# CrawlScript/tf_geometric

Measured on AMD Instinct MI355X. Metric: aggregated edges/sec + achieved HBM GB/s, GCN layer, higher is better.
Workload: dtype f32

## Files before the change

### tf_geometric_amd/csrc/tfgx_reduce.hip

```cpp
#include "tfgx_common.h"
#include <cfloat>
#include <cstdio>
#include <cstdlib>

namespace tfgx {
namespace {

template <int G>
__device__ __forceinline__ int bcast_i(int v, int j)
{
    if constexpr (G == 64) return __builtin_amdgcn_readlane(v, j);
    else return __shfl(v, j, G);
}
template <int G>
__device__ __forceinline__ float bcast_f(float v, int j)
{
    if constexpr (G == 64) return __int_as_float(__builtin_amdgcn_readlane(__float_as_int(v), j));
    else return __shfl(v, j, G);
}

struct KArgs {
    const int32_t* row_begin;
    const int32_t* row_end;
    int64_t rp_stride;
// ... 286 lines not shown
                            if constexpr (IS_MAX) {
                                const float m = WEIGHTED ? xv[u][k][v] * ww[u] : xv[u][k][v];
                                if constexpr (TRACK) {
                                    if (live) track_step(k, v, m, base + j + u);
                                }
                                const float t = fmaxf(acc[k][v], m);
                                acc[k][v] = live ? t : acc[k][v];
                            } else {
                                const float t = WEIGHTED ? fmaf(ww[u], xv[u][k][v], acc[k][v]) : acc[k][v] + xv[u][k][v];
                                acc[k][v] = live ? t : acc[k][v];
                            }
                        }
                }
            }
            }
        }

        const float sc = a.self_coef ? a.self_coef[r] : 0.0f;
        bool mismatch = false;
        float divisor = 1.0f;
        if (a.op == TFGX_MEAN) {
            const int cnt = a.mean_count ? a.mean_count[r] : (e - s);
            divisor = float(cnt > 1 ? cnt : 1);
        }
#pragma unroll
        for (int k = 0; k < CH; ++k) {
            if (!cvalid[k]) continue;
            float res[VEC];
#pragma unroll
            for (int v = 0; v < VEC; ++v) res[v] = acc[k][v];
            float* op = a.out + r * a.ldo + coff[k];
            float mine[TRACK ? VEC : 1], before[TRACK ? VEC : 1];
            if (a.accumulate) {
                float prev[VEC];
                load_vec<VEC>(op, prev);
#pragma unroll
                for (int v = 0; v < VEC; ++v) {
                    if constexpr (TRACK) { mine[v] = res[v]; before[v] = prev[v]; }
                    res[v] = IS_MAX ? fmaxf(prev[v], res[v]) : prev[v] + res[v];
                }
            }
            if (a.self_coef) {
                float xself[VEC];
                if constexpr (VERIFY) {
                    float xlay[VEC];
                    load_vec<VEC>(a.verify_x + r * a.ld_verify_x + coff[k], xself);
                    load_vec<VEC>(xs[k] + r * xsl[k], xlay);
#pragma unroll
                    for (int v = 0; v < VEC; ++v) mismatch = mismatch || __float_as_uint(xself[v]) != __float_as_uint(xlay[v]);
                } else if constexpr (SPLIT) load_vec<VEC>(xs[k] + r * xsl[k], xself);
                else load_vec<VEC>(a.x + r * a.ldx + coff[k], xself);
#pragma unroll
                for (int v = 0; v < VEC; ++v) {
                    if constexpr (IS_MAX) res[v] = fmaxf(res[v], sc * xself[v]);
                    else res[v] = fmaf(sc, xself[v], res[v]);
                }
            }
            if (a.op == TFGX_MEAN) {
#pragma unroll
                for (int v = 0; v < VEC; ++v) res[v] = res[v] / divisor;
            }
            if (a.add_x) {
                float xa[VEC];
                load_vec<VEC>(a.add_x + r * a.ld_add + coff[k], xa);
#pragma unroll
                for (int v = 0; v < VEC; ++v) res[v] = xa[v] + res[v];
            }
            if (a.bias) {
                float b[VEC];
                load_vec<VEC>(a.bias + coff[k], b);
#pragma unroll
                for (int v = 0; v < VEC; ++v) res[v] += b[v];
            }
#pragma unroll
            for (int v = 0; v < VEC; ++v) res[v] = apply_act(res[v], a.act);
            store_vec<VEC>(op, res);
            if constexpr (TRACK) {
                const int s_rel = a.track_row_begin ? a.track_row_begin[r * a.rp_stride] : s;
                uint32_t pk[VEC];
#pragma unroll
                for (int v = 0; v < VEC; ++v) {
                    const uint32_t c = uint32_t(tcnt[k][v] < 65535 ? tcnt[k][v] : 65535);
                    pk[v] = (c << 16) | (tpos[k][v] < 0 ? 0xFFFFu : uint32_t(tpos[k][v] - s_rel) & 0xFFFFu);
                }
                uint32_t* tp = a.track + r * a.ld_track + coff[k];
                if (a.accumulate) {
                    uint32_t old[VEC];
                    if constexpr (VEC == 4) {
                        const uint4 o4 = *reinterpret_cast<const uint4*>(tp);
                        old[0] = o4.x; old[1] = o4.y; old[2] = o4.z; old[3] = o4.w;
                    } else {
#pragma unroll
                        for (int v = 0; v < VEC; ++v) old[v] = tp[v];
                    }
#pragma unroll
                    for (int v = 0; v < VEC; ++v) {
                        const uint32_t oc = old[v] >> 16, nc = pk[v] >> 16;
                        const uint32_t sum = oc + nc < 65535u ? oc + nc : 65535u;
                        const bool none_before = (old[v] & 0xFFFFu) == 0xFFFFu && oc == 0u;
                        if (mine[v] > before[v] || none_before) {  }
                        else if (mine[v] == before[v] && nc > 0u) pk[v] = (sum << 16) | (old[v] & 0xFFFFu);
                        else pk[v] = old[v];
                    }
                }
                if constexpr (VEC == 4) *reinterpret_cast<uint4*>(tp) = make_uint4(pk[0], pk[1], pk[2], pk[3]);
                else {
#pragma unroll
                    for (int v = 0; v < VEC; ++v) tp[v] = pk[v];
                }
            }
        }
        if constexpr (VERIFY) {
            if (mismatch) *a.verify_word = 1u;
        }
    }
}

inline size_t dummy_lds_bytes()
{
    static long v = -1;
    if (v < 0) {
        const char* e = getenv("TFGX_REDUCE_DUMMY_LDS");
        v = (e != nullptr && atol(e) > 0) ? atol(e) : 0;
    }
    return size_t(v);
}

inline int reduce_grid_cap()
{
    static int cap = 0;
    if (cap == 0) {
        const char* e = getenv("TFGX_REDUCE_GRID_CAP");
        cap = (e != nullptr && atoi(e) > 0) ? atoi(e) : TFGX_REDUCE_GRID_CAP_DEFAULT;
    }
    return cap;
}

inline bool wide_blocks_enabled()
{
    static int v = -1;
    if (v < 0) {
        const char* e = getenv("TFGX_REDUCE_WIDE_BLOCKS");
        v = (e != nullptr && atoi(e) == 0) ? 0 : 1;
    }
    return v != 0;
}
inline int wide_g256()
{
    static int v = -1;
    if (v < 0) {
        const char* e = getenv("TFGX_REDUCE_WIDE_G256");
        v = (e != nullptr && atoi(e) == 16) ? 16 : 32;
    }
    return v;
}

template <int VEC, int G, int CH, int U = 0>
int launch_cfg(const KArgs& a, bool is_max, bool weighted, int ny, hipStream_t stream)
{
    constexpr int ROWS_PER_BLOCK = kBlock / G;
    dim3 grid(grid_for(a.n_dst, ROWS_PER_BLOCK, CH >= 2 ? (reduce_grid_cap() < 4096 ? reduce_grid_cap() : 4096) : reduce_grid_cap()), ny, 1);
    dim3 block(kBlock, 1, 1);
    if constexpr (VEC == 4 && CH == 1) {
        if (a.x_tail != nullptr && a.verify_x != nullptr) {
            if (is_max) {
                if (weighted) seg_reduce_verify_kernel<VEC, G, CH, true, true, U><<<grid, block, dummy_lds_bytes(), stream>>>(a);
                else seg_reduce_verify_kernel<VEC, G, CH, true, false, U><<<grid, block, dummy_lds_bytes(), stream>>>(a);
            } else {
                if (weighted) seg_reduce_verify_kernel<VEC, G, CH, false, true, U><<<grid, block, dummy_lds_bytes(), stream>>>(a);
                else seg_reduce_verify_kernel<VEC, G, CH, false, false, U><<<grid, block, dummy_lds_bytes(), stream>>>(a);
            }
            TFGX_LAUNCH_CHECK("seg_reduce_verify_kernel");
            return TFGX_OK;
        }
        if (a.x_tail != nullptr) {
            if (is_max) {
                if (weighted) seg_reduce_kernel<VEC, G, CH, true, true, true, false, U><<<grid, block, dummy_lds_bytes(), stream>>>(a);
                else seg_reduce_kernel<VEC, G, CH, true, false, true, false, U><<<grid, block, dummy_lds_bytes(), stream>>>(a);
            } else {
                if (weighted) seg_reduce_kernel<VEC, G, CH, false, true, true, false, U><<<grid, block, dummy_lds_bytes(), stream>>>(a);
                else seg_reduce_kernel<VEC, G, CH, false, false, true, false, U><<<grid, block, dummy_lds_bytes(), stream>>>(a);
            }
            TFGX_LAUNCH_CHECK("seg_reduce_kernel<split>");
            return TFGX_OK;
        }
    }
    if (a.x_tail != nullptr) {
        set_error("tfgx_segment_reduce_f32: x_tail needs 16-byte aligned rows and F <= 256");
        return TFGX_ERR_INVALID_ARG;
    }
    if (a.track != nullptr) {
        if constexpr (VEC == 4 && CH == 1) {
            if (weighted) seg_reduce_kernel<VEC, G, CH, true, true, false, true, U><<<grid, block, dummy_lds_bytes(), stream>>>(a);
            else seg_reduce_kernel<VEC, G, CH, true, false, false, true, U><<<grid, block, dummy_lds_bytes(), stream>>>(a);
            TFGX_LAUNCH_CHECK("seg_reduce_kernel<track>");
            return TFGX_OK;
        }
        set_error("tfgx_segment_reduce_f32: track needs 16-byte aligned rows, F % 4 == 0, of F <= 256 columns or of whole 128-byte lines");
        return TFGX_ERR_INVALID_ARG;
    }
    if (is_max) {
        if (weighted) seg_reduce_kernel<VEC, G, CH, true, true, false, false, U><<<grid, block, dummy_lds_bytes(), stream>>>(a);
        else seg_reduce_kernel<VEC, G, CH, true, false, false, false, U><<<grid, block, dummy_lds_bytes(), stream>>>(a);
    } else {
        if (weighted) seg_reduce_kernel<VEC, G, CH, false, true, false, false, U><<<grid, block, dummy_lds_bytes(), stream>>>(a);
        else seg_reduce_kernel<VEC, G, CH, false, false, false, false, U><<<grid, block, dummy_lds_bytes(), stream>>>(a);
    }
    TFGX_LAUNCH_CHECK("seg_reduce_kernel");
    return TFGX_OK;
}

template <typename K>
int resident_grid(K k, int* blocks)
{
    if (*blocks == 0) {
        int dev = 0, cus = 0, per_cu = 0;
        if (hipGetDevice(&dev) != hipSuccess ||
            hipDeviceGetAttribute(&cus, hipDeviceAttributeMultiprocessorCount, dev) != hipSuccess || cus <= 0)
            cus = 256;
        if (hipOccupancyMaxActiveBlocksPerMultiprocessor(&per_cu, k, kBlock, 0) != hipSuccess || per_cu <= 0) per_cu = 1;
        *blocks = cus * per_cu;
    }
    return *blocks;
}

template <int G>
int launch_repair_g(const KArgs& a, bool is_max, bool weighted, hipStream_t stream)
{
    static int blocks[4] = {0, 0, 0, 0};
    auto go = [&](auto kernel, int slot) {
        kernel<<<dim3(resident_grid(kernel, &blocks[slot]), 1, 1), dim3(kBlock, 1, 1), 0, stream>>>(a);
    };
    if (is_max) {
        if (weighted) go(seg_reduce_repair_kernel<4, G, 1, true, true>, 0);
        else go(seg_reduce_repair_kernel<4, G, 1, true, false>, 1);
    } else {
        if (weighted) go(seg_reduce_repair_kernel<4, G, 1, false, true>, 2);
        else go(seg_reduce_repair_kernel<4, G, 1, false, false>, 3);
    }
    TFGX_LAUNCH_CHECK("seg_reduce_repair_kernel");
    return TFGX_OK;
}

int launch_repair(const KArgs& a, int G, bool is_max, bool weighted, hipStream_t stream)
{
    switch (G) {
        case 4: return launch_repair_g<4>(a, is_max, weighted, stream);
        case 8: return launch_repair_g<8>(a, is_max, weighted, stream);
        case 16: return launch_repair_g<16>(a, is_max, weighted, stream);
        case 32: return launch_repair_g<32>(a, is_max, weighted, stream);
        default: return launch_repair_g<64>(a, is_max, weighted, stream);
    }
}

struct GroupShape { int G, CH, NY, U; };

inline GroupShape group_shape(const KArgs& a, int vec)
{
    const int lanes = (a.F + vec - 1) / vec;
    if (vec == 4 && a.F >= 128 && a.F % 32 == 0 && a.ldx % 32 == 0 && aligned_to(a.x, 128) && a.x_tail == nullptr &&
        a.wide_blocks >= 0 && (a.wide_blocks > 0 || wide_blocks_enabled())) {
        const int g = a.F == 256 ? wide_g256() : 16;
        return GroupShape{g, 1, (lanes + g - 1) / g, 16};
    }
    if (lanes <= 4) return GroupShape{4, 1, 1, 0};
    if (lanes <= 8) return GroupShape{8, 1, 1, 0};
    if (lanes <= 16) return GroupShape{16, 1, 1, 0};
    if (lanes <= 32) return GroupShape{32, 1, 1, 0};
    if (lanes <= 64) return GroupShape{64, 1, 1, 0};
    if (lanes <= 128) return GroupShape{64, 2, 1, 0};
    const int per = 64 * 4;
    return GroupShape{64, 4, (lanes + per - 1) / per, 0};
}

template <int VEC>
int launch_vec(const KArgs& a, bool is_max, bool weighted, hipStream_t stream)
{
    const GroupShape g = group_shape(a, VEC);
    if constexpr (VEC == 4) {
        if (g.U == 16 && g.G == 16) return launch_cfg<4, 16, 1, 16>(a, is_max, weighted, g.NY, stream);
        if (g.U == 16 && g.G == 32) return launch_cfg<4, 32, 1, 16>(a, is_max, weighted, g.NY, stream);
    }
    if (g.CH == 1) {
        switch (g.G) {
            case 4: return launch_cfg<VEC, 4, 1>(a, is_max, weighted, 1, stream);
            case 8: return launch_cfg<VEC, 8, 1>(a, is_max, weighted, 1, stream);
            case 16: return launch_cfg<VEC, 16, 1>(a, is_max, weighted, 1, stream);
            case 32: return launch_cfg<VEC, 32, 1>(a, is_max, weighted, 1, stream);
            default: return launch_cfg<VEC, 64, 1>(a, is_max, weighted, 1, stream);
        }
    }
    if (g.CH == 2) return launch_cfg<VEC, 64, 2>(a, is_max, weighted, 1, stream);
    return launch_cfg<VEC, 64, 4>(a, is_max, weighted, g.NY, stream);
}

struct HubArgs {
    const int32_t* hub_rows;
    const int32_t* hub_chunk_ptr;
    const float* scratch;
    int64_t n_hub;
    KArgs k;
};

__global__ __launch_bounds__(kBlock) void hub_finalize_kernel(const HubArgs h)
{
    const KArgs& a = h.k;
    const bool is_max = a.op == TFGX_MAX;
    int64_t t = blockIdx.x * int64_t(kBlock) + threadIdx.x;
    const int64_t stride = int64_t(gridDim.x) * kBlock;
    const int64_t total = h.n_hub * a.F;
    for (; t < total; t += stride) {
        const int64_t i = t / a.F;
        const int j = int(t - i * a.F);
        const int64_t r = h.hub_rows[i];
        float res = is_max ? -FLT_MAX : 0.0f;
        constexpr int HB = 16;
        int c = h.hub_chunk_ptr[i];
        const int c_end = h.hub_chunk_ptr[i + 1];
        const float* sp = h.scratch + int64_t(c) * a.F + j;
        for (; c + HB <= c_end; c += HB, sp += int64_t(HB) * a.F) {
            float v[HB];
#pragma unroll
            for (int u = 0; u < HB; ++u) v[u] = __builtin_nontemporal_load(sp + int64_t(u) * a.F);
#pragma unroll
            for (int u = 0; u < HB; ++u) res = is_max ? fmaxf(res, v[u]) : res + v[u];
        }
        for (; c < c_end; ++c, sp += a.F) {
            const float v = *sp;
            res = is_max ? fmaxf(res, v) : res + v;
        }
        float* op = a.out + r * a.ldo + j;
        if (a.accumulate) res = is_max ? fmaxf(*op, res) : *op + res;
        if (a.self_coef) {
            const float xv = (a.x_tail != nullptr && j >= a.f_main) ? a.x_tail[r * a.ld_tail + (j - a.f_main)]
                                                                    : a.x[r * a.ldx + j];
            res = is_max ? fmaxf(res, a.self_coef[r] * xv) : fmaf(a.self_coef[r], xv, res);
        }
        if (a.op == TFGX_MEAN) {
            const int cnt = a.mean_count ? a.mean_count[r]
                                         : (a.row_end[r * a.rp_stride] - a.row_begin[r * a.rp_stride]);
            res = res / float(cnt > 1 ? cnt : 1);
        }
        if (a.add_x) res = a.add_x[r * a.ld_add + j] + res;
        if (a.bias) res += a.bias[j];
        *op = apply_act(res, a.act);
    }
}

int launch_any(const KArgs& a, int vec, bool is_max, bool weighted, hipStream_t stream)
{
    if (vec == 4) return launch_vec<4>(a, is_max, weighted, stream);
    if (vec == 2) return launch_vec<2>(a, is_max, weighted, stream);
    return launch_vec<1>(a, is_max, weighted, stream);
}

}
}

using namespace tfgx;

static int vector_width(const tfgx_reduce_args* p)
{
    auto ok = [&](int vec) {
        const size_t al = sizeof(float) * vec;
        bool good = (p->F % vec == 0) && (p->ldx % vec == 0) && (p->ldo % vec == 0) && aligned_to(p->x, al) &&
                    aligned_to(p->out, al);
        if (p->add_x) good = good && (p->ld_add % vec == 0) && aligned_to(p->add_x, al);
        if (p->bias) good = good && aligned_to(p->bias, al);
        return good;
    };
    int vec = ok(4) ? 4 : (ok(2) ? 2 : 1);
    while (vec > 1 && p->F / vec < 8) vec /= 2;
    return vec;
}

extern "C" int tfgx_segment_reduce_describe(const tfgx_reduce_args* p, char* buf, size_t buf_bytes)
{
    TFGX_REQUIRE(p != nullptr && buf != nullptr && buf_bytes > 0, "null argument");
    const int vec = vector_width(p);
    KArgs a;
    a.F = int32_t(p->F); a.ldx = p->ldx; a.x = p->x; a.x_tail = p->x_tail; a.wide_blocks = p->wide_blocks;
    const GroupShape g = group_shape(a, vec);
    const bool split = p->x_tail != nullptr && vec == 4 && g.CH == 1;
    if (p->verify && split) {
        const bool fused = p->self_coef != nullptr && p->n_verify == p->n_dst;
        snprintf(buf, buf_bytes, "%sseg_reduce_verify_kernel<%d, %d, %d, %s, %s, %d> + seg_reduce_repair_kernel",
                 fused ? "" : "split_rows_compare_kernel + ", vec, g.G, g.CH, p->op == TFGX_MAX ? "true" : "false",
                 p->w ? "true" : "false", g.U);
        return TFGX_OK;
    }
    snprintf(buf, buf_bytes, "seg_reduce_kernel<%d, %d, %d, %s, %s, %s, %s, %d>", vec, g.G, g.CH, p->op == TFGX_MAX ? "true" : "false",
             p->w ? "true" : "false", split ? "true" : "false", p->track ? "true" : "false", g.U);
    return TFGX_OK;
}

extern "C" int tfgx_segment_reduce_f32(const tfgx_reduce_args* p, tfgx_stream_t stream_)
{
    TFGX_RANGE();
    TFGX_REQUIRE(p != nullptr, "args is null");
    TFGX_REQUIRE(p->n_dst >= 0 && p->F >= 1 && p->F < (int64_t(1) << 30), "bad n_dst / F");
    TFGX_REQUIRE(p->op == TFGX_SUM || p->op == TFGX_MEAN || p->op == TFGX_MAX, "bad op");
    TFGX_REQUIRE(p->act == TFGX_ACT_NONE || p->act == TFGX_ACT_RELU, "bad act");
    if (p->n_dst == 0) return TFGX_OK;
    TFGX_REQUIRE(p->row_begin && p->row_end && p->out && p->x, "null pointer");
    TFGX_REQUIRE((p->ldx >= p->F || p->x_tail) && p->ldo >= p->F, "leading dimension < F");
    TFGX_REQUIRE(p->rp_stride >= 1, "rp_stride < 1");
    TFGX_REQUIRE(!(p->add_x) || p->ld_add >= p->F, "ld_add < F");

    KArgs a;
    a.row_begin = p->row_begin; a.row_end = p->row_end; a.rp_stride = p->rp_stride;
    a.col = p->col; a.w = p->w; a.n_dst = p->n_dst; a.x = p->x; a.ldx = p->ldx; a.F = int32_t(p->F);
    a.col0 = 0; a.out = p->out; a.ldo = p->ldo; a.op = p->op; a.act = p->act; a.accumulate = p->accumulate;
    a.self_coef = p->self_coef; a.bias = p->bias; a.add_x = p->add_x; a.ld_add = p->ld_add;
    a.mean_count = p->mean_count;
    a.hub_threshold = 0;
    a.x_tail = p->x_tail; a.ld_tail = p->ld_tail; a.f_main = int32_t(p->f_main);
    a.edge_tail = p->edge_tail; a.ld_edge_tail = p->ld_edge_tail;
    a.wide_blocks = p->wide_blocks;
    a.row_order = p->row_order;
    a.track = p->track; a.ld_track = p->ld_track; a.track_row_begin = p->track_row_begin;
    if (p->track) {
        TFGX_REQUIRE(p->op == TFGX_MAX && !p->self_coef && !p->x_tail && p->hub_threshold == 0 && !p->bias && !p->add_x &&
                         p->act == TFGX_ACT_NONE,
                     "track: plain TFGX_MAX launches only (no self_coef / bias / activation / split rows / hub lists)");
        TFGX_REQUIRE(p->ld_track >= p->F && p->ld_track % 4 == 0 && aligned_to(p->track, 16), "track: bad leading dimension / alignment");
    }
    TFGX_REQUIRE(p->edge_tail == nullptr ||
                     (p->x_tail != nullptr && p->ld_edge_tail >= p->F - p->f_main && p->ld_edge_tail % 4 == 0 &&
                      aligned_to(p->edge_tail, 16)),
                 "edge_tail needs the split-row layout (x_tail) and 16-byte aligned rows");
    if (p->x_tail) {
        TFGX_REQUIRE(p->f_main > 0 && p->f_main < p->F && p->f_main % 4 == 0 && (p->F - p->f_main) % 4 == 0 &&
                         p->ld_tail >= p->F - p->f_main && p->ld_tail % 4 == 0 && p->ldx >= p->f_main &&
                         aligned_to(p->x_tail, 16),
                     "bad split-row layout (f_main / ld_tail / alignment)");
    }
    const bool use_hub = p->hub_threshold > 0 && p->n_hub_rows > 0;
    if (use_hub) {
        TFGX_REQUIRE(p->hub_rows && p->hub_chunk_ptr && p->hub_chunk_begin && p->hub_chunk_end && p->hub_scratch &&
                         p->n_hub_chunks > 0,
                     "hub rows given without chunk lists / scratch");
        a.hub_threshold = p->hub_threshold;
    }

    const bool is_max = p->op == TFGX_MAX;
    const bool weighted = p->w != nullptr;
    hipStream_t stream = as_stream(stream_);

    int vec = vector_width(p);
    a.verify_x = nullptr; a.ld_verify_x = 0; a.verify_word = nullptr;
    if (p->verify) {
        TFGX_REQUIRE(p->x_tail && p->edge_tail && p->verify_x && p->verify_word && p->n_verify >= 0,
                     "verify: needs the split layout with edge_tail, verify_x and verify_word");
        TFGX_REQUIRE(!p->accumulate && !p->track && !use_hub, "verify: no accumulate / track / hub lists");
        TFGX_REQUIRE(p->ld_verify_x >= p->F && p->ld_verify_x % 4 == 0 && aligned_to(p->verify_x, 16) &&
                         aligned_to(p->verify_word, 4),
                     "verify: verify_x needs 16-byte aligned rows");
        const GroupShape g = group_shape(a, vec);
        TFGX_REQUIRE(vec == 4 && g.CH == 1, "verify: the split layout needs 16-byte aligned rows and F <= 256");
        a.verify_word = p->verify_word;
        if (p->self_coef != nullptr && p->n_verify == p->n_dst) {
            a.verify_x = p->verify_x;
            a.ld_verify_x = p->ld_verify_x;
        } else if (p->n_verify > 0) {
            split_rows_compare_kernel<<<grid_for(p->n_verify * (p->F / 4), kBlock, 8192), kBlock, 0, stream>>>(
                p->verify_x, p->ld_verify_x, p->n_verify, int(p->F), int(p->f_main), p->x, p->ldx, p->x_tail, p->ld_tail,
                p->verify_word);
            TFGX_LAUNCH_CHECK("split_rows_compare_kernel");
        }
        int rc = launch_any(a, vec, is_max, weighted, stream);
        if (rc != TFGX_OK) return rc;
        KArgs r = a;
        r.x = p->verify_x; r.ldx = p->ld_verify_x; r.x_tail = nullptr; r.ld_tail = 0; r.f_main = 0;
        r.edge_tail = nullptr; r.ld_edge_tail = 0; r.verify_x = nullptr; r.ld_verify_x = 0;
        return launch_repair(r, g.G, is_max, weighted, stream);
    }
    int rc = launch_any(a, vec, is_max, weighted, stream);
    if (rc != TFGX_OK || !use_hub) return rc;

    KArgs c = a;
    c.row_begin = p->hub_chunk_begin; c.row_end = p->hub_chunk_end; c.rp_stride = 1;
    c.n_dst = p->n_hub_chunks; c.out = p->hub_scratch; c.ldo = p->F;
    c.op = is_max ? TFGX_MAX : TFGX_SUM; c.act = TFGX_ACT_NONE; c.accumulate = 0;
    c.self_coef = nullptr; c.bias = nullptr; c.add_x = nullptr; c.mean_count = nullptr; c.hub_threshold = 0;
    c.row_order = nullptr; c.track = nullptr; c.track_row_begin = nullptr;
    const bool sok = (p->F % 4 == 0) && aligned_to(p->hub_scratch, 16) && (p->ldx % 4 == 0) && aligned_to(p->x, 16);
    const bool sok2 = (p->F % 2 == 0) && aligned_to(p->hub_scratch, 8) && (p->ldx % 2 == 0) && aligned_to(p->x, 8);
    rc = launch_any(c, sok ? 4 : (sok2 ? 2 : 1), is_max, weighted, stream);
    if (rc != TFGX_OK) return rc;
    HubArgs h;
    h.hub_rows = p->hub_rows; h.hub_chunk_ptr = p->hub_chunk_ptr; h.scratch = p->hub_scratch;
    h.n_hub = p->n_hub_rows; h.k = a;
    hub_finalize_kernel<<<grid_for(p->n_hub_rows * p->F, kBlock), kBlock, 0, stream>>>(h);
    TFGX_LAUNCH_CHECK("hub_finalize_kernel");
    return TFGX_OK;
}
```

### tf_geometric_amd/plan.py

```python
import ctypes

import torch

from . import _lib as L

CACHE_KEY_PLAN = "tfgx_csr_plan"


class CsrPlan(object):

    def __init__(self, row_ptr, col, perm, n_dst, n_src, num_edges):
        self.row_ptr = row_ptr
        self.col = col
        self.perm = perm
        self.n_dst = int(n_dst)
        self.n_src = int(n_src)
        self.num_edges = int(num_edges)
        self._edge_index = None
        self._transposed = None
        self._hub = None

    @staticmethod
    def build(edge_index, n_dst, n_src=None):
        lib = L.require_gpu()
# ... 389 lines not shown
CACHE_KEY_STATIC_ROWS = "tfgx_static_rows"


STATIC_STATS = {"hits": 0, "builds": 0}


def _static_key(x, plan):
    return (x.data_ptr(), x._version, int(x.shape[0]), int(x.shape[1]), id(plan))


def _build_static_rows(x, plan, cache):
    n, F = int(x.shape[0]), int(x.shape[1])
    rows, nbytes = None, 0
    if SplitRows.wanted(n, F):
        rows = SplitRows.from_dense(x).with_edge_tail(plan)
        nbytes = 4 * (rows.main.numel() + rows.tail.numel() + rows.edge_tail.numel())
    cache[CACHE_KEY_STATIC_ROWS] = (_static_key(x, plan), rows, x, plan, nbytes)
    STATIC_STATS["builds"] += 1
    return rows, nbytes


CACHE_KEY_STATIC_AGG = "tfgx_static_aggregated"


def prepare_static_features(x, edge_index, cache, num_nodes=None, cache_aggregation=False):
    if cache is None:
        raise ValueError("prepare_static_features needs the graph's cache dict")
    x = L.as_f32(x)
    if x.dim() != 2 or not x.is_contiguous():
        raise ValueError("static features must be a contiguous [num_nodes, num_features] float32 tensor")
    n = int(x.shape[0]) if num_nodes is None else int(num_nodes)
    plan = edge_index if isinstance(edge_index, CsrPlan) else CsrPlan.from_cache(edge_index, n, int(x.shape[0]), cache)
    cache[CACHE_KEY_STATIC] = x
    cache.pop(CACHE_KEY_STATIC_AUTO, None)
    if cache_aggregation:
        cache[CACHE_KEY_STATIC_AGG] = {}
    else:
        cache.pop(CACHE_KEY_STATIC_AGG, None)
    rows, nbytes = _build_static_rows(x, plan, cache)
    F = int(x.shape[1])
    return dict(bytes=nbytes, layout="edge_tail" if rows is not None else "dense", tensor=x,
                f_main=(F // 32) * 32 if rows is not None else F, f_tail=F % 32 if rows is not None else 0)


def release_static_features(cache):
    cache.pop(CACHE_KEY_STATIC_AUTO, None)
    cache.pop(CACHE_KEY_STATIC, None)
    cache.pop(CACHE_KEY_STATIC_ROWS, None)
    cache.pop(CACHE_KEY_STATIC_AGG, None)


def _declared_static(x, cache):
    if cache is None or not isinstance(x, torch.Tensor):
        return False
    opt = cache.get(CACHE_KEY_STATIC, None)
    if opt is None or opt is False or not isinstance(opt, torch.Tensor):
        return False
    return (opt.data_ptr() == x.data_ptr() and opt.shape == x.shape and opt.dtype == x.dtype
            and opt.stride() == x.stride())


def static_aggregate(x, plan, cache, op, w_csr=None, self_coef=None):
    store = cache.get(CACHE_KEY_STATIC_AGG) if cache is not None else None
    if store is None or not _declared_static(x, cache):
        return None
    if any(t is not None and t.requires_grad for t in (x, w_csr, self_coef)):
        return None
    if torch.cuda.is_current_stream_capturing():
        return None
    ident = lambda t: None if t is None else (t.data_ptr(), t._version, int(t.numel()))
    key = (_static_key(x, plan), ident(w_csr), ident(self_coef))
    hit = store.get(op)
    if hit is not None and hit[0] == key:
        STATIC_STATS["agg_hits"] = STATIC_STATS.get("agg_hits", 0) + 1
        return hit[1]
    out = segment_reduce(plan, static_rows(x, plan, cache), op, w_csr=w_csr, self_coef=self_coef)
    store[op] = (key, out, x, w_csr, self_coef)
    return out


def static_aggregate_applies(x, cache):
    store = cache.get(CACHE_KEY_STATIC_AGG) if cache is not None else None
    return store is not None and _declared_static(x, cache) and not torch.cuda.is_current_stream_capturing()


import os as _os
import weakref as _weakref

AUTO_STATIC_LAYOUT = _os.environ.get("TFGX_STATIC_LAYOUT", "auto") != "explicit"
CACHE_KEY_STATIC_SEEN = "tfgx_static_seen"
CACHE_KEY_STATIC_AUTO = "tfgx_static_auto"
CACHE_KEY_STATIC_DISTRUST = "tfgx_static_distrust"
_AGG_LAUNCHES = [0]


_AUTO_SUPPRESSED = [0]


class no_auto_promotion(object):

    def __enter__(self):
        _AUTO_SUPPRESSED[0] += 1
        return self

    def __exit__(self, *exc):
        _AUTO_SUPPRESSED[0] -= 1
        return False


def written_by_kernel(t):
    if isinstance(t, torch.Tensor):
        torch.autograd.graph.increment_version(t)
    return t


def static_layout_budget_bytes():
    env = _os.environ.get("TFGX_STATIC_LAYOUT_BUDGET")
    if env is not None:
        return int(float(env))
    free, _ = torch.cuda.mem_get_info()
    return free // 10


def _auto_promote(x, plan, cache):
    if (not AUTO_STATIC_LAYOUT or _AUTO_SUPPRESSED[0] > 0 or x.dim() != 2 or not x.is_contiguous() or x.requires_grad or x.dtype != torch.float32
            or not x.is_cuda or not SplitRows.wanted(int(x.shape[0]), int(x.shape[1]))
            or torch.cuda.is_current_stream_capturing()):
        return False
    bad = cache.get(CACHE_KEY_STATIC_DISTRUST)
    if bad is not None and bad() is x.untyped_storage():
        return False
    seen = cache.setdefault(CACHE_KEY_STATIC_SEEN, {})
    key = _static_key(x, plan)
    store = x.untyped_storage()
    hit = seen.get(x.data_ptr())
    if hit is None or hit[0]() is not store or hit[1] != key:
        if len(seen) >= 8:
            seen.clear()
        seen[x.data_ptr()] = (_weakref.ref(store), key, _AGG_LAUNCHES[0])
        return False
    if _AGG_LAUNCHES[0] == hit[2]:
        return False
    F = int(x.shape[1])
    need = 4 * (int(x.shape[0]) * F + plan.num_edges * (F % 32))
    if need > static_layout_budget_bytes():
        return False
    seen.pop(x.data_ptr(), None)
    cache[CACHE_KEY_STATIC] = x
    cache[CACHE_KEY_STATIC_AUTO] = True
    STATIC_STATS["auto_promotions"] = STATIC_STATS.get("auto_promotions", 0) + 1
    STATIC_STATS["auto_promoted_bytes"] = need
    import logging
    logging.getLogger("tf_geometric_amd").info(
        "static feature layout: tensor [%d, %d] seen unchanged twice -> split + edge-tail copy of %.2f GB held in the graph's "
        "cache (TFGX_STATIC_LAYOUT=explicit turns this off; tfg.release_static_features(cache) frees it)",
        int(x.shape[0]), F, need / 1e9)
    return True


_VERIFY_CALLS = [0]


def _verify_rows_setting():
    v = _os.environ.get("TFGX_STATIC_VERIFY_ROWS", "4096")
    return -1 if v == "all" else max(int(v), 0)


def _promoted_layout_is_current(x, rows):
    samples = _verify_rows_setting()
    if samples == 0:
        return True
    n, F = int(x.shape[0]), int(x.shape[1])
    if samples < 0:
        samples = n
    lib = L.require_gpu()
    flag = torch.empty(1, dtype=torch.int32, device=x.device)
    _VERIFY_CALLS[0] += 1
    L.check(lib.tfgx_split_rows_verify_f32(L.ptr(x), int(x.stride(0)), n, F, int(rows.main.shape[1]), L.ptr(rows.main), int(rows.main.stride(0)),
                                           L.ptr(rows.tail), int(rows.tail.stride(0)), samples,
                                           (0x5DEECE66D * _VERIFY_CALLS[0] + 11) & 0xFFFFFFFFFFFFFFFF, L.ptr(flag), L.stream_ptr()),
            "tfgx_split_rows_verify_f32")
    STATIC_STATS["verifications"] = STATIC_STATS.get("verifications", 0) + 1
    return int(flag.item()) == 0


def static_rows(x, plan, cache):
    if cache is None or not isinstance(x, torch.Tensor):
        return x
    opt = cache.get(CACHE_KEY_STATIC, None)
    auto = bool(cache.get(CACHE_KEY_STATIC_AUTO))
    if auto and torch.cuda.is_current_stream_capturing():
        return x
    same = isinstance(opt, torch.Tensor) and (opt.data_ptr() == x.data_ptr() and opt.shape == x.shape and
                                              opt.dtype == x.dtype and opt.stride() == x.stride())
    if not same:
        if (opt is None or (auto and isinstance(opt, torch.Tensor))) and _auto_promote(x, plan, cache):
            cache.pop(CACHE_KEY_STATIC_ROWS, None)
            cache.pop(CACHE_KEY_STATIC_AGG, None)
        else:
            return x
    hit = cache.get(CACHE_KEY_STATIC_ROWS)
    if hit is not None and hit[0] == _static_key(x, plan):
        if hit[1] is not None and cache.get(CACHE_KEY_STATIC_AUTO) and not _promoted_layout_is_current(x, hit[1]):
            release_static_features(cache)
            STATIC_STATS["auto_demotions"] = STATIC_STATS.get("auto_demotions", 0) + 1
            STATIC_STATS["stale_copies_caught"] = STATIC_STATS.get("stale_copies_caught", 0) + 1
            cache[CACHE_KEY_STATIC_DISTRUST] = _weakref.ref(x.untyped_storage())
            return x
        if hit[1] is not None:
            STATIC_STATS["hits"] += 1
        return x if hit[1] is None else hit[1]
    if torch.cuda.is_current_stream_capturing() or x.dim() != 2 or not x.is_contiguous():
        return x
    if hit is not None and cache.get(CACHE_KEY_STATIC_AUTO):
        release_static_features(cache)
        STATIC_STATS["auto_demotions"] = STATIC_STATS.get("auto_demotions", 0) + 1
        _auto_promote(x, plan, cache)
        return x
    rows, _ = _build_static_rows(x, plan, cache)
    return x if rows is None else rows


def edge_weight_csr(plan, edge_weight, cache=None):
    if edge_weight is None:
        return None
    ver = edge_weight._version if isinstance(edge_weight, torch.Tensor) else None
    if cache is not None:
        hit = cache.get("tfgx_edge_weight_csr")
        if hit is not None and hit[0] is edge_weight and hit[2] is plan and hit[3] == ver:
            return hit[1]
    w_csr = plan.edge_attr_to_csr(edge_weight)
    if cache is not None:
        cache["tfgx_edge_weight_csr"] = (edge_weight, w_csr, plan, ver)
    return w_csr


RELAY_POW2_TABLES = True


def relaid_for_gather(x, ldx, plan_is_skewed, dry_run=False):
    F = int(x.shape[1])
    if not (RELAY_POW2_TABLES and ldx == F and pow2_row_stride(F) and (F >= 512 or plan_is_skewed)):
        return x, ldx
    n = int(x.shape[0])
    need = 4 * n * (F + 32)
    if 4 * n * F <= (512 << 20):
        return x, ldx
    capturing = torch.cuda.is_current_stream_capturing()
    key = (x.data_ptr(), n, F)
    hit = None if capturing else _RELAID.get(key)
    if hit is not None:
        storage_ref, version, wide = hit
        if storage_ref() is not None and version == x._version and _relaid_copy_is_current(x, wide, F):
            if not dry_run:
                RELAY_STATS["hits"] = RELAY_STATS.get("hits", 0) + 1
            return wide[:, :F], F + 32
        _RELAID.pop(key, None)
        if storage_ref() is not None and version == x._version:
            RELAY_STATS["stale_copies_caught"] = RELAY_STATS.get("stale_copies_caught", 0) + 1
        del wide, hit
    free, _ = torch.cuda.mem_get_info()
    if need > free // 2:
        return x, ldx
    if dry_run:
        return x, F + 32
    wide = torch.empty((n, F + 32), dtype=torch.float32, device=x.device)
    L.check(L.require_gpu().tfgx_gather_rows_f32(L.ptr(x), ldx, None, n, F, L.ptr(wide), F + 32, L.stream_ptr()),
            "tfgx_gather_rows_f32 (strided row copy)")
    RELAY_STATS["copies"] += 1
    if not capturing:
        while len(_RELAID) >= 2:
            _RELAID.pop(next(iter(_RELAID)))
        _RELAID[key] = (_weakref.ref(x.untyped_storage()), x._version, wide)
    return wide[:, :F], F + 32


RELAY_STATS = {"copies": 0}
_RELAID = {}


def _relaid_copy_is_current(x, wide, F):
    samples = _verify_rows_setting()
    if samples == 0:
        return True
    n = int(x.shape[0])
    if samples < 0:
        samples = n
    half = (F // 2) // 4 * 4
    lib = L.require_gpu()
    flag = torch.empty(1, dtype=torch.int32, device=x.device)
    _VERIFY_CALLS[0] += 1
    L.check(lib.tfgx_split_rows_verify_f32(L.ptr(x), int(x.stride(0)), n, F, half, L.ptr(wide), int(wide.stride(0)),
                                           wide.data_ptr() + 4 * half, int(wide.stride(0)), samples,
                                           (0x5DEECE66D * _VERIFY_CALLS[0] + 11) & 0xFFFFFFFFFFFFFFFF, L.ptr(flag), L.stream_ptr()),
            "tfgx_split_rows_verify_f32 (re-laid copy)")
    return int(flag.item()) == 0


def release_relaid_copies():
    _RELAID.clear()


VERIFIED_STATS = {"promotions": 0, "served": 0, "demotions": 0}


class _LayoutMemo(dict):
    """data_ptr -> _VerifiedLayout of one plan (a dict type that finalizers can refer to weakly)."""


class _VerifiedLayout(object):
    __slots__ = ("store", "key", "rows", "word", "seen", "demoted", "__weakref__")

    def __init__(self, store, key):
        self.store, self.key = _weakref.ref(store), key
        self.rows = self.word = self.seen = None
        self.demoted = False

    def drop(self):
        self.rows = self.word = self.seen = None


def _forget_layout(memo_ref, ptr, ent_ref):
    memo, ent = memo_ref(), ent_ref()
    if memo is not None and ent is not None and memo.get(ptr) is ent:
        del memo[ptr]
        ent.drop()


def verified_layout(plan, x, describe=False):
    if (not AUTO_STATIC_LAYOUT or _AUTO_SUPPRESSED[0] > 0 or not isinstance(x, torch.Tensor) or x.dim() != 2
            or not x.is_cuda or x.dtype != torch.float32 or x.requires_grad or not x.is_contiguous() or x.data_ptr() % 16
            or not SplitRows.wanted(int(x.shape[0]), int(x.shape[1])) or torch.cuda.is_current_stream_capturing()
            or plan.hub_info() is not None):
        return None
    memo = plan.__dict__.get("_verified")
    if memo is None:
        if describe:
            return None
        memo = plan._verified = _LayoutMemo()
    store = x.untyped_storage()
    ptr, key = x.data_ptr(), (x._version, int(x.shape[0]), int(x.shape[1]))
    ent = memo.get(ptr)
    if ent is not None and ent.store() is not store:
        ent = None
    if describe:
        return ent if ent is not None and ent.rows is not None and ent.key == key and not ent.demoted else None
    if ent is None:
        if len(memo) >= 8:
            for p in [p for p, e in memo.items() if e.rows is None and not e.demoted]:
                del memo[p]
        ent = memo[ptr] = _VerifiedLayout(store, key)
        _weakref.finalize(store, _forget_layout, _weakref.ref(memo), ptr, _weakref.ref(ent))
        return None
    if ent.demoted:
        return None
    if ent.key != key:
        ent.drop()
        ent.key = key
        return None
    if ent.rows is None:
        F = int(x.shape[1])
        need = 4 * (int(x.shape[0]) * F + plan.num_edges * (F % 32))
        if need > static_layout_budget_bytes():
            return None
        ent.rows = SplitRows.from_dense(x).with_edge_tail(plan)
        ent.word = torch.zeros(1, dtype=torch.int32, device=x.device)
        ent.seen = torch.zeros(1, dtype=torch.int32, pin_memory=True)
        VERIFIED_STATS["promotions"] += 1
    elif int(ent.seen[0]) != 0:
        ent.drop()
        ent.demoted = True
        VERIFIED_STATS["demotions"] += 1
        return None
    return ent


def wide_blocks_hint(explicit_spans, has_hub_lists, ldx, num_edges, n_rows):
    if explicit_spans:
        return -1
    if not has_hub_lists and num_edges < 32 * max(int(n_rows), 1):
        return -1
    if has_hub_lists and not pow2_row_stride(ldx):
        return -1
    return 0


def segment_reduce(plan, x, op, w_csr=None, out=None, act=L.ACT_NONE, self_coef=None, bias=None, add_x=None,
                   accumulate=False, mean_count=None, row_begin=None, row_end=None, rp_stride=1, col=None,
                   n_dst=None, describe=False, track=None, track_row_begin=None, wide_blocks=None, out_dtype=None):
    if isinstance(x, HalfRows):
        if track is not None or track_row_begin is not None:
            raise L.TfgxError("tfgx_segment_reduce_h16: track: not supported on a 16-bit table (max aggregation is inference-only)")
        return _segment_reduce_h16(plan, x, op, w_csr, out, act, self_coef, bias, add_x, accumulate, mean_count, row_begin,
                                   row_end, rp_stride, col, n_dst, describe, wide_blocks, out_dtype)
    if out_dtype not in (None, torch.float32):
        raise TypeError("segment_reduce: out_dtype needs a HalfRows input")
    lib = L.require_gpu()
    split = x if isinstance(x, SplitRows) else None
    verified = None
    if (split is None and row_begin is None and row_end is None and col is None and track is None and not accumulate
            and (n_dst is None or int(n_dst) == plan.n_dst)):
        verified = verified_layout(plan, x, describe=describe)
        if verified is not None:
            table, split = x, verified.rows
    if split is not None:
        x, ldx = L.row_major_2d(split.main)
        F = split.shape[1]
    else:
        x, ldx = L.row_major_2d(x)
        F = int(x.shape[1])
        if row_begin is None and row_end is None and col is None:
            x, ldx = relaid_for_gather(x, ldx, plan.hub_info() is not None, dry_run=describe)
    n_dst = plan.n_dst if n_dst is None else int(n_dst)
    given = out is not None
    if out is None:
        out = torch.empty((n_dst, F), dtype=torch.float32, device=x.device)
    out2, ldo = L.row_major_2d(out)
    assert out2 is out, "out must be row-major"
    a = L.ReduceArgs()
    rb = plan.row_ptr if row_begin is None else row_begin
    re = plan.row_ptr[1:] if row_end is None else row_end
    a.row_begin = rb.data_ptr()
    a.row_end = re.data_ptr()
    a.rp_stride = rp_stride
    c = plan.col if col is None else col
    a.col = c.data_ptr()
    a.w = 0 if w_csr is None else w_csr.data_ptr()
    a.n_dst = n_dst
    a.x = x.data_ptr()
    a.ldx = ldx
    a.F = F
    a.out = out.data_ptr()
    a.ldo = ldo
    a.op = op
    a.act = act
    a.accumulate = 1 if accumulate else 0
    a.self_coef = 0 if self_coef is None else self_coef.data_ptr()
    a.bias = 0 if bias is None else bias.data_ptr()
    if add_x is not None:
        add_x, ld_add = L.row_major_2d(add_x)
        a.add_x = add_x.data_ptr()
        a.ld_add = ld_add
    a.mean_count = 0 if mean_count is None else mean_count.data_ptr()
    if split is not None:
        a.x_tail, a.ld_tail, a.f_main = split.tail.data_ptr(), int(split.tail.shape[1]), int(split.main.shape[1])
        if split.edge_tail is not None and split.edge_plan is plan and col is None:
            a.edge_tail, a.ld_edge_tail = split.edge_tail.data_ptr(), int(split.edge_tail.shape[1])
    if verified is not None:
        a.verify, a.verify_x, a.ld_verify_x = 1, table.data_ptr(), int(table.stride(0))
        a.n_verify, a.verify_word = int(table.shape[0]), verified.word.data_ptr()
    if row_begin is None and row_end is None and col is None and n_dst == plan.n_dst and USE_ROW_ORDER and F <= ROW_ORDER_MAX_F:
        order = plan.row_order()
        if order is not None:
            a.row_order = order.data_ptr()
    if track is not None:
        a.track, a.ld_track = track.data_ptr(), int(track.stride(0))
        if track_row_begin is not None:
            a.track_row_begin = track_row_begin.data_ptr()
    hub = plan.hub_info() if (row_begin is None and row_end is None and col is None and track is None
                              and n_dst == plan.n_dst) else None
    if hub is not None:
        hub_rows, chunk_ptr, chunk_begin, chunk_end, _ = hub
        scratch = torch.empty((int(chunk_begin.shape[0]), F), dtype=torch.float32, device=x.device)
        a.hub_threshold = plan.hub_threshold
        a.hub_rows, a.hub_chunk_ptr = hub_rows.data_ptr(), chunk_ptr.data_ptr()
        a.hub_chunk_begin, a.hub_chunk_end = chunk_begin.data_ptr(), chunk_end.data_ptr()
        a.n_hub_rows, a.n_hub_chunks = int(hub_rows.shape[0]), int(chunk_begin.shape[0])
        a.hub_scratch = scratch.data_ptr()
    a.wide_blocks = wide_blocks_hint(explicit_spans=row_begin is not None or row_end is not None or col is not None,
                                     has_hub_lists=hub is not None, ldx=ldx, num_edges=plan.num_edges, n_rows=n_dst)
    if wide_blocks is not None:
        a.wide_blocks = int(wide_blocks)
    if describe:
        buf = ctypes.create_string_buffer(160)
        L.check(lib.tfgx_segment_reduce_describe(ctypes.byref(a), buf, 160), "tfgx_segment_reduce_describe")
        return buf.value.decode()
    L.check(lib.tfgx_segment_reduce_f32(ctypes.byref(a), L.stream_ptr()), "tfgx_segment_reduce_f32")
    _AGG_LAUNCHES[0] += 1
    if verified is not None:
        verified.seen.copy_(verified.word, non_blocking=True)
        VERIFIED_STATS["served"] += 1
    if given:
        written_by_kernel(out)
    if track is not None:
        written_by_kernel(track)
    return out


FUSE_AGGREGATE_GEMM = True
TFGX_FUSE_WIDE = False


FUSED_STATS = {"launches": 0, "with_side_output": 0}


def aggregate_gemm_applies(x, kernel, op=L.SUM):
    if not FUSE_AGGREGATE_GEMM or op not in (L.SUM, L.MEAN) or kernel is None:
        return False
    lib = L.require_gpu()
    x2, ldx = L.row_major_2d(x.main if isinstance(x, SplitRows) else x)
    F, N = (x.shape[1] if isinstance(x, SplitRows) else int(x2.shape[1])), int(kernel.shape[1])
    return bool(int(kernel.shape[0]) == F and lib.tfgx_aggregate_gemm_fits(F, N) and ldx % 4 == 0
                and x2.data_ptr() % 16 == 0)


def aggregate_gemm(plan, x, op, kernel, w_csr=None, self_coef=None, bias=None, act=L.ACT_NONE, out=None, agg_out=None):
    if not FUSE_AGGREGATE_GEMM or op not in (L.SUM, L.MEAN):
        return None
    lib = L.require_gpu()
    split = x if isinstance(x, SplitRows) else None
    x2, ldx = L.row_major_2d(split.main if split is not None else x)
    k2, ldb = L.row_major_2d(L.as_f32(kernel))
    F, N = (split.shape[1] if split is not None else int(x2.shape[1])), int(k2.shape[1])
    if int(k2.shape[0]) != F or not lib.tfgx_aggregate_gemm_fits(F, N) or ldx % 4 != 0 or x2.data_ptr() % 16 != 0:
        return None
    hub = plan.hub_info()
    order = plan.row_order()
    if (split is None and agg_out is None and hub is None and F >= 128 and F % 32 == 0 and ldx % 32 == 0 and x2.data_ptr() % 128 == 0
            and plan.num_edges >= 32 * max(plan.n_dst, 1) and 4 * int(x2.shape[0]) * F > (512 << 20) and not TFGX_FUSE_WIDE):
        return None
    if split is None:
        x2, ldx = relaid_for_gather(x2, ldx, hub is not None)
    n_dst = plan.n_dst
    given = out is not None
    if out is None:
        out = torch.empty((n_dst, N), dtype=torch.float32, device=x2.device)
    _, ldc = L.row_major_2d(out)
    a = L.ReduceArgs()
    a.row_begin, a.row_end, a.rp_stride = plan.row_ptr.data_ptr(), plan.row_ptr[1:].data_ptr(), 1
    a.col = plan.col.data_ptr()
    a.w = 0 if w_csr is None else w_csr.data_ptr()
    a.n_dst, a.x, a.ldx, a.F = n_dst, x2.data_ptr(), ldx, F
    a.op = op
    a.self_coef = 0 if self_coef is None else self_coef.data_ptr()
    if split is not None:
        a.x_tail, a.ld_tail, a.f_main = split.tail.data_ptr(), int(split.tail.shape[1]), int(split.main.shape[1])
        if split.edge_tail is not None and split.edge_plan is plan:
            a.edge_tail, a.ld_edge_tail = split.edge_tail.data_ptr(), int(split.edge_tail.shape[1])
    if order is not None:
        a.row_order = order.data_ptr()
    if hub is not None:
        hub_rows, chunk_ptr, chunk_begin, chunk_end, _ = hub
        scratch = torch.empty((int(chunk_begin.shape[0]), F), dtype=torch.float32, device=x2.device)
        a.hub_threshold = plan.hub_threshold
        a.hub_rows, a.hub_chunk_ptr = hub_rows.data_ptr(), chunk_ptr.data_ptr()
        a.hub_chunk_begin, a.hub_chunk_end = chunk_begin.data_ptr(), chunk_end.data_ptr()
        a.n_hub_rows, a.n_hub_chunks = int(hub_rows.shape[0]), int(chunk_begin.shape[0])
        a.hub_scratch = scratch.data_ptr()
        slot = plan.hub_order_slot()
        if slot is not None:
            a.hub_order_slot = slot.data_ptr()
    if agg_out is not None:
        ao, ldo = L.row_major_2d(agg_out)
        assert ao is agg_out and tuple(agg_out.shape) == (n_dst, F) and ldo % 4 == 0 and agg_out.data_ptr() % 16 == 0
        a.out, a.ldo = agg_out.data_ptr(), ldo
        FUSED_STATS["with_side_output"] += 1
    FUSED_STATS["launches"] += 1
    _AGG_LAUNCHES[0] += 1
    bias_t = None if bias is None else L.as_f32(bias).contiguous()
    L.check(lib.tfgx_aggregate_gemm_f32(ctypes.byref(a), L.ptr(k2), ldb, L.ptr(bias_t), act, L.ptr(out), ldc, N,
                                        L.stream_ptr()), "tfgx_aggregate_gemm_f32")
    if given:
        written_by_kernel(out)
    written_by_kernel(agg_out)
    return out


def can_track(plan, x2, ldx):
    F = int(x2.shape[1])
    wide = (F % 32 == 0 and ldx % 32 == 0 and x2.data_ptr() % 128 == 0 and _os.environ.get("TFGX_REDUCE_WIDE_BLOCKS", "1") != "0"
            and plan.num_edges >= 32 * max(plan.n_dst, 1))
    return (F % 4 == 0 and F >= 32 and (F <= 256 or wide) and ldx % 4 == 0 and x2.data_ptr() % 16 == 0 and plan.hub_info() is None
            and int(getattr(plan, "hub_threshold", 1 << 30)) < 65536)


def _avg_lines(F, ld):
    import math
    row, stride = 4 * F, 4 * ld
    period = 128 // math.gcd(stride, 128)
    return sum(((i * stride) % 128 + row - 1) // 128 + 1 for i in range(period)) / period


def gather_friendly_ld(F):
    F = int(F)
    if F <= 0:
        return max(F, 1)
    cands = [F, (F + 15) // 16 * 16, (F + 31) // 32 * 32]
    if F <= 32:
        cands.append(1 << (F - 1).bit_length())
    best = min(sorted(set(cands)), key=lambda ld: (round(_avg_lines(F, ld), 6), ld))
    if pow2_row_stride(best):
        best += 32
    return best


def pow2_row_stride(ld):
    ld = int(ld)
    return ld >= 128 and (ld & (ld - 1)) == 0


def gather_friendly_empty(n, F, device):
    ld = gather_friendly_ld(F)
    buf = torch.empty((int(n), ld), dtype=torch.float32, device=device)
    return buf if ld == int(F) else buf[:, :int(F)]


def gather_friendly_copy(t):
    F = int(t.shape[1])
    if t.stride(1) == 1 and t.stride(0) == gather_friendly_ld(F):
        return t
    if gather_friendly_ld(F) == F:
        return t.contiguous()
    out = gather_friendly_empty(int(t.shape[0]), F, t.device)
    out.copy_(t)
    return out


def gemm_bias_act(a, b, bias=None, act=L.ACT_NONE, out=None, act_cols=None):
    lib = L.require_gpu()
    a, lda = L.row_major_2d(L.as_f32(a))
    b, ldb = L.row_major_2d(L.as_f32(b))
    M, K = int(a.shape[0]), int(a.shape[1])
    if int(b.shape[0]) != K:
        raise ValueError("matmul shape mismatch: {} @ {}".format(tuple(a.shape), tuple(b.shape)))
    N = int(b.shape[1])
    given = out is not None
    if out is None:
        out = torch.empty((M, N), dtype=torch.float32, device=a.device)
    _, ldc = L.row_major_2d(out)
    bias_t = None if bias is None else L.as_f32(bias).contiguous()
    ws_bytes = lib.tfgx_gemm_workspace_bytes(M, K, N)
    ws = torch.empty(ws_bytes, dtype=torch.uint8, device=a.device) if ws_bytes else None
    L.check(lib.tfgx_gemm_bias_act_cols_ws_f32(L.ptr(a), lda, L.ptr(b), ldb, L.ptr(bias_t), act,
                                               N if act_cols is None else int(act_cols), L.ptr(out), ldc, M, K, N,
                                               L.ptr(ws), ws_bytes, L.stream_ptr()), "tfgx_gemm_bias_act_cols_ws_f32")
    if given:
        written_by_kernel(out)
    return out


def l2_normalize_rows_(h):
    lib = L.require_gpu()
    h2, ld = L.row_major_2d(h)
    assert h2 is h
    L.check(lib.tfgx_l2_normalize_rows_f32(L.ptr(h), ld, int(h.shape[0]), int(h.shape[1]), L.stream_ptr()),
            "tfgx_l2_normalize_rows_f32")
    return h


def gather_rows(x, idx, out=None):
    lib = L.require_gpu()
    x, ldx = L.row_major_2d(x)
    idx = L.as_i32(idx)
    M, F = int(idx.shape[0]), int(x.shape[1])
    given = out is not None
    if out is None:
        out = torch.empty((M, F), dtype=torch.float32, device=x.device)
    _, ldo = L.row_major_2d(out)
    L.check(lib.tfgx_gather_rows_f32(L.ptr(x), ldx, L.ptr(idx), M, F, L.ptr(out), ldo, L.stream_ptr()),
            "tfgx_gather_rows_f32")
    if given:
        written_by_kernel(out)
    return out


def gemm_tn(x, g, want_bias=False, gate=None):
    lib = L.require_gpu()
    x, ldx = L.row_major_2d(L.as_f32(x))
    g, ldg = L.row_major_2d(L.as_f32(g))
    M, Ka, N = int(x.shape[0]), int(x.shape[1]), int(g.shape[1])
    if int(g.shape[0]) != M:
        raise ValueError("gemm_tn: x has {} rows, g has {}".format(M, int(g.shape[0])))
    ldt = 0
    if gate is not None:
        gate, ldt = L.row_major_2d(gate)
        if tuple(gate.shape) != (M, N):
            raise ValueError("gemm_tn: gate has shape {}, g has {}".format(tuple(gate.shape), (M, N)))
    dW = torch.empty((Ka, N), dtype=torch.float32, device=x.device)
    db = torch.empty(N, dtype=torch.float32, device=x.device) if want_bias else None
    ws_bytes = lib.tfgx_gemm_tn_workspace_bytes(M, Ka, N, 1 if want_bias else 0)
    ws = torch.empty(max(ws_bytes, 1), dtype=torch.uint8, device=x.device)
    L.check(lib.tfgx_gemm_tn_gated_f32(L.ptr(x), ldx, L.ptr(g), ldg, L.ptr(gate), ldt, M, Ka, N, L.ptr(dW), N, L.ptr(db),
                                       L.ptr(ws), ws_bytes, L.stream_ptr()), "tfgx_gemm_tn_gated_f32")
    return dW, db


def column_sums(g):
    lib = L.require_gpu()
    g2, ldg = L.row_major_2d(L.as_f32(g))
    M, N = int(g2.shape[0]), int(g2.shape[1])
    out = torch.empty(N, dtype=torch.float32, device=g2.device)
    ws_bytes = lib.tfgx_column_sum_workspace_bytes(M, N)
    ws = torch.empty(max(ws_bytes, 1), dtype=torch.uint8, device=g2.device)
    L.check(lib.tfgx_column_sum_f32(L.ptr(g2), ldg, M, N, L.ptr(out), L.ptr(ws), ws_bytes, L.stream_ptr()), "tfgx_column_sum_f32")
    return out


def transpose(a):
    lib = L.require_gpu()
    a, lda = L.row_major_2d(L.as_f32(a))
    r, c = int(a.shape[0]), int(a.shape[1])
    out = torch.empty((c, r), dtype=torch.float32, device=a.device)
    L.check(lib.tfgx_transpose_f32(L.ptr(a), lda, r, c, L.ptr(out), r, L.stream_ptr()), "tfgx_transpose_f32")
    return out
```

Baseline: 15.66 billion.

## Allow verified split-row layout on plans with hub-row chunk lists

Extends the verified static split-row layout path so it can run when the plan has hub rows. It adds a verify-aware hub finalize kernel that checks self-term inputs against the reference copy, plus conditional repair kernels for the chunks and the finalize step that exit early when the verify word is clear. This lets hub-heavy graphs use the cheaper split layout for gathers instead of falling back to the plain path. In exchange it adds several extra launches per call (repair launches that return early) and more host-side branching.

```diff
diff --git a/tf_geometric_amd/csrc/tfgx_reduce.hip b/tf_geometric_amd/csrc/tfgx_reduce.hip
--- a/tf_geometric_amd/csrc/tfgx_reduce.hip
+++ b/tf_geometric_amd/csrc/tfgx_reduce.hip
@@ -612,7 +612,8 @@
     KArgs k;
 };
 
-__global__ __launch_bounds__(kBlock) void hub_finalize_kernel(const HubArgs h)
+template <bool VERIFY>
+__device__ __forceinline__ void hub_finalize_walk(const HubArgs& h)
 {
     const KArgs& a = h.k;
     const bool is_max = a.op == TFGX_MAX;
@@ -642,8 +643,13 @@
         float* op = a.out + r * a.ldo + j;
         if (a.accumulate) res = is_max ? fmaxf(*op, res) : *op + res;
         if (a.self_coef) {
-            const float xv = (a.x_tail != nullptr && j >= a.f_main) ? a.x_tail[r * a.ld_tail + (j - a.f_main)]
-                                                                    : a.x[r * a.ldx + j];
+            float xv = (a.x_tail != nullptr && j >= a.f_main) ? a.x_tail[r * a.ld_tail + (j - a.f_main)]
+                                                              : a.x[r * a.ldx + j];
+            if constexpr (VERIFY) {
+                const float xt = a.verify_x[r * a.ld_verify_x + j];
+                if (__float_as_uint(xt) != __float_as_uint(xv)) *a.verify_word = 1u;
+                xv = xt;
+            }
             res = is_max ? fmaxf(res, a.self_coef[r] * xv) : fmaf(a.self_coef[r], xv, res);
         }
         if (a.op == TFGX_MEAN) {
@@ -655,6 +661,22 @@
         if (a.bias) res += a.bias[j];
         *op = apply_act(res, a.act);
     }
+}
+
+__global__ __launch_bounds__(kBlock) void hub_finalize_kernel(const HubArgs h)
+{
+    hub_finalize_walk<false>(h);
+}
+
+__global__ __launch_bounds__(kBlock) void hub_finalize_verify_kernel(const HubArgs h)
+{
+    hub_finalize_walk<true>(h);
+}
+
+__global__ __launch_bounds__(kBlock) void hub_finalize_repair_kernel(const HubArgs h)
+{
+    if (*h.k.verify_word == 0u) return;
+    hub_finalize_walk<false>(h);
 }
 
 int launch_any(const KArgs& a, int vec, bool is_max, bool weighted, hipStream_t stream)
@@ -694,9 +716,12 @@
     const bool split = p->x_tail != nullptr && vec == 4 && g.CH == 1;
     if (p->verify && split) {
         const bool fused = p->self_coef != nullptr && p->n_verify == p->n_dst;
-        snprintf(buf, buf_bytes, "%sseg_reduce_verify_kernel<%d, %d, %d, %s, %s, %d> + seg_reduce_repair_kernel",
+        const bool hub = p->hub_threshold > 0 && p->n_hub_rows > 0;
+        snprintf(buf, buf_bytes, "%sseg_reduce_verify_kernel<%d, %d, %d, %s, %s, %d>%s + %s",
                  fused ? "" : "split_rows_compare_kernel + ", vec, g.G, g.CH, p->op == TFGX_MAX ? "true" : "false",
-                 p->w ? "true" : "false", g.U);
+                 p->w ? "true" : "false", g.U,
+                 !hub ? "" : (fused ? " + hub chunks<split> + hub_finalize_verify_kernel" : " + hub chunks<split> + hub_finalize_kernel"),
+                 hub ? "3 repair launches" : "seg_reduce_repair_kernel");
         return TFGX_OK;
     }
     snprintf(buf, buf_bytes, "seg_reduce_kernel<%d, %d, %d, %s, %s, %s, %s, %d>", vec, g.G, g.CH, p->op == TFGX_MAX ? "true" : "false",
@@ -758,18 +783,33 @@
     hipStream_t stream = as_stream(stream_);
 
     int vec = vector_width(p);
+    auto chunk_args = [&](const KArgs& k) {
+        KArgs c = k;
+        c.row_begin = p->hub_chunk_begin; c.row_end = p->hub_chunk_end; c.rp_stride = 1;
+        c.n_dst = p->n_hub_chunks; c.out = p->hub_scratch; c.ldo = p->F;
+        c.op = is_max ? TFGX_MAX : TFGX_SUM; c.act = TFGX_ACT_NONE; c.accumulate = 0;
+        c.self_coef = nullptr; c.bias = nullptr; c.add_x = nullptr; c.mean_count = nullptr; c.hub_threshold = 0;
+        c.row_order = nullptr; c.track = nullptr; c.track_row_begin = nullptr;
+        c.verify_x = nullptr; c.ld_verify_x = 0;
+        return c;
+    };
+    HubArgs h;
+    h.hub_rows = p->hub_rows; h.hub_chunk_ptr = p->hub_chunk_ptr; h.scratch = p->hub_scratch;
+    h.n_hub = p->n_hub_rows;
     a.verify_x = nullptr; a.ld_verify_x = 0; a.verify_word = nullptr;
     if (p->verify) {
         TFGX_REQUIRE(p->x_tail && p->edge_tail && p->verify_x && p->verify_word && p->n_verify >= 0,
                      "verify: needs the split layout with edge_tail, verify_x and verify_word");
-        TFGX_REQUIRE(!p->accumulate && !p->track && !use_hub, "verify: no accumulate / track / hub lists");
+        TFGX_REQUIRE(!p->accumulate && !p->track, "verify: no accumulate / track");
         TFGX_REQUIRE(p->ld_verify_x >= p->F && p->ld_verify_x % 4 == 0 && aligned_to(p->verify_x, 16) &&
                          aligned_to(p->verify_word, 4),
                      "verify: verify_x needs 16-byte aligned rows");
         const GroupShape g = group_shape(a, vec);
         TFGX_REQUIRE(vec == 4 && g.CH == 1, "verify: the split layout needs 16-byte aligned rows and F <= 256");
+        TFGX_REQUIRE(!use_hub || aligned_to(p->hub_scratch, 16), "verify: hub_scratch needs 16-byte alignment");
         a.verify_word = p->verify_word;
-        if (p->self_coef != nullptr && p->n_verify == p->n_dst) {
+        const bool fused = p->self_coef != nullptr && p->n_verify == p->n_dst;
+        if (fused) {
             a.verify_x = p->verify_x;
             a.ld_verify_x = p->ld_verify_x;
         } else if (p->n_verify > 0) {
@@ -783,24 +823,34 @@
         KArgs r = a;
         r.x = p->verify_x; r.ldx = p->ld_verify_x; r.x_tail = nullptr; r.ld_tail = 0; r.f_main = 0;
         r.edge_tail = nullptr; r.ld_edge_tail = 0; r.verify_x = nullptr; r.ld_verify_x = 0;
-        return launch_repair(r, g.G, is_max, weighted, stream);
+        if (!use_hub) return launch_repair(r, g.G, is_max, weighted, stream);
+
+        rc = launch_any(chunk_args(a), 4, is_max, weighted, stream);
+        if (rc != TFGX_OK) return rc;
+        h.k = a;
+        const int fin_grid = grid_for(p->n_hub_rows * p->F, kBlock);
+        if (fused) hub_finalize_verify_kernel<<<fin_grid, kBlock, 0, stream>>>(h);
+        else hub_finalize_kernel<<<fin_grid, kBlock, 0, stream>>>(h);
+        TFGX_LAUNCH_CHECK("hub_finalize_kernel (verified route)");
+        rc = launch_repair(r, g.G, is_max, weighted, stream);
+        if (rc != TFGX_OK) return rc;
+        rc = launch_repair(chunk_args(r), g.G, is_max, weighted, stream);
+        if (rc != TFGX_OK) return rc;
+        h.k = r;
+        static int fin_blocks = 0;
+        const int rep_grid = resident_grid(hub_finalize_repair_kernel, &fin_blocks);
+        hub_finalize_repair_kernel<<<rep_grid < fin_grid ? rep_grid : fin_grid, kBlock, 0, stream>>>(h);
+        TFGX_LAUNCH_CHECK("hub_finalize_repair_kernel");
+        return TFGX_OK;
     }
     int rc = launch_any(a, vec, is_max, weighted, stream);
     if (rc != TFGX_OK || !use_hub) return rc;
 
-    KArgs c = a;
-    c.row_begin = p->hub_chunk_begin; c.row_end = p->hub_chunk_end; c.rp_stride = 1;
-    c.n_dst = p->n_hub_chunks; c.out = p->hub_scratch; c.ldo = p->F;
-    c.op = is_max ? TFGX_MAX : TFGX_SUM; c.act = TFGX_ACT_NONE; c.accumulate = 0;
-    c.self_coef = nullptr; c.bias = nullptr; c.add_x = nullptr; c.mean_count = nullptr; c.hub_threshold = 0;
-    c.row_order = nullptr; c.track = nullptr; c.track_row_begin = nullptr;
     const bool sok = (p->F % 4 == 0) && aligned_to(p->hub_scratch, 16) && (p->ldx % 4 == 0) && aligned_to(p->x, 16);
     const bool sok2 = (p->F % 2 == 0) && aligned_to(p->hub_scratch, 8) && (p->ldx % 2 == 0) && aligned_to(p->x, 8);
-    rc = launch_any(c, sok ? 4 : (sok2 ? 2 : 1), is_max, weighted, stream);
+    rc = launch_any(chunk_args(a), sok ? 4 : (sok2 ? 2 : 1), is_max, weighted, stream);
     if (rc != TFGX_OK) return rc;
-    HubArgs h;
-    h.hub_rows = p->hub_rows; h.hub_chunk_ptr = p->hub_chunk_ptr; h.scratch = p->hub_scratch;
-    h.n_hub = p->n_hub_rows; h.k = a;
+    h.k = a;
     hub_finalize_kernel<<<grid_for(p->n_hub_rows * p->F, kBlock), kBlock, 0, stream>>>(h);
     TFGX_LAUNCH_CHECK("hub_finalize_kernel");
     return TFGX_OK;
diff --git a/tf_geometric_amd/plan.py b/tf_geometric_amd/plan.py
--- a/tf_geometric_amd/plan.py
+++ b/tf_geometric_amd/plan.py
@@ -715,6 +715,7 @@
 
 
 VERIFIED_STATS = {"promotions": 0, "served": 0, "demotions": 0}
+VERIFIED_LAYOUT_ON_HUB_PLANS = True
 
 
 class _LayoutMemo(dict):
@@ -744,7 +745,7 @@
     if (not AUTO_STATIC_LAYOUT or _AUTO_SUPPRESSED[0] > 0 or not isinstance(x, torch.Tensor) or x.dim() != 2
             or not x.is_cuda or x.dtype != torch.float32 or x.requires_grad or not x.is_contiguous() or x.data_ptr() % 16
             or not SplitRows.wanted(int(x.shape[0]), int(x.shape[1])) or torch.cuda.is_current_stream_capturing()
-            or plan.hub_info() is not None):
+            or (not VERIFIED_LAYOUT_ON_HUB_PLANS and plan.hub_info() is not None)):
         return None
     memo = plan.__dict__.get("_verified")
     if memo is None:
@@ -885,8 +886,8 @@
     if wide_blocks is not None:
         a.wide_blocks = int(wide_blocks)
     if describe:
-        buf = ctypes.create_string_buffer(160)
-        L.check(lib.tfgx_segment_reduce_describe(ctypes.byref(a), buf, 160), "tfgx_segment_reduce_describe")
+        buf = ctypes.create_string_buffer(192)
+        L.check(lib.tfgx_segment_reduce_describe(ctypes.byref(a), buf, 192), "tfgx_segment_reduce_describe")
         return buf.value.decode()
     L.check(lib.tfgx_segment_reduce_f32(ctypes.byref(a), L.stream_ptr()), "tfgx_segment_reduce_f32")
     _AGG_LAUNCHES[0] += 1
```

Result: no change. 15.66 billion, median of 2 (-0.0%).
